# slp-rl/aero

Hardware: NVIDIA H100
Metric: audio-seconds/sec forward (higher is better)
Workload: dtype f16 tensor-core operands and activation storage (10-bit mantissa = tf32), fp32 accumulate / norm inputs / cell state

## Files before the change

aero_b200/csrc/tapgemm.cuh:

```cuda
#pragma once
#include <cuda.h>
#include "common.cuh"

namespace aero {
struct TapGemmArgs {
    const void* a1;
    const void* a2;
    const void* w;
    const float* bias;
    const float* addend_fn;
    const float* colscale;
    const void* residual;
    const float* samp_affine;
    void* out;
    double* stats;
    aero_tapgemm_params p;
    int ntaps;
    int tiles_t;
    int ldw;
    int vec_a;
    int vec_o;
    int vec_o8;
    uint32_t dv_mul[3], dv_shr[3];
    int direct_f16;
    int direct_f32;
    int last_tile;
};
constexpr int kBM = 128;
constexpr int kMaxStages = 8;
constexpr int kMaxBN = 128;
constexpr int kWideBN = 256;
constexpr int kSliceBN = 64;
constexpr int kProducerRegs = 40, kConsumerRegs = 232;
constexpr int kEpiWarps = 8;
constexpr int kThreads = 128 + 32 * kEpiWarps;
constexpr int kATileBytes = kBM * 128;

struct TcShared {
    uint64_t full[kMaxStages];
    uint64_t empty[kMaxStages];
    float stats[kEpiWarps][8][2];
    float part[kEpiWarps][4][2];
    alignas(16) float stage[kEpiWarps][32][20];
};

using KernelFn = void (*)(CUtensorMap, CUtensorMap, CUtensorMap, TapGemmArgs, int, int, int);
int tapgemm_simt_launch(const TapGemmArgs& g, cudaStream_t st);
int tapgemm_tc_launch(const TapGemmArgs& g, cudaStream_t st);
bool tapgemm_tc_eligible(const aero_tapgemm_params& p);
}
```

aero_b200/csrc/tapgemm_tc.cu:

```cuda
#include <cuda.h>
#include <mutex>
#include <unordered_map>
#include <string>
#include <cstring>
#include <cstdlib>

#include "tapgemm.cuh"
#include "tc_common.cuh"

namespace aero {

KernelFn tapgemm_tc_kernels_bn32(bool f16a, bool f16o, int amode, bool res, bool stats);
KernelFn tapgemm_tc_kernels_bn64(bool f16a, bool f16o, int amode, bool res, bool stats);
KernelFn tapgemm_tc_kernels_bn96(bool f16a, bool f16o, int amode, bool res, bool stats);
KernelFn tapgemm_tc_kernels_bn128(bool f16a, bool f16o, int amode, bool res, bool stats);
KernelFn tapgemm_tc_kernels_bn192(bool f16a, bool f16o, int amode, bool res, bool stats);
KernelFn tapgemm_tc_kernels_bn256(bool f16a, bool f16o, int amode, bool res, bool stats);

typedef CUresult (*EncodeTiledFn)(CUtensorMap*, CUtensorMapDataType, cuuint32_t, void*, const cuuint64_t*, const cuuint64_t*,
                                  const cuuint32_t*, const cuuint32_t*, CUtensorMapInterleave, CUtensorMapSwizzle,
                                  CUtensorMapL2promotion, CUtensorMapFloatOOBfill);

static EncodeTiledFn get_encode() {
    static EncodeTiledFn fn = nullptr;
// ... 18 lines not shown
    size_t operator()(const MapKey& k) const {
        const uint64_t* w = reinterpret_cast<const uint64_t*>(&k);
        size_t h = 1469598103934665603ull;
        for (size_t i = 0; i < sizeof(MapKey) / 8; ++i) h = (h ^ w[i]) * 1099511628211ull;
        return h;
    }
};

int encode_map(CUtensorMap* out, const void* base, uint32_t rank, const uint64_t* dims, const uint64_t* strides_bytes,
               const uint32_t* box, int swizzle_mode, int elem_bytes) {
    static std::mutex mu;
    static std::unordered_map<MapKey, CUtensorMap, MapKeyHash> cache;
    MapKey key;
    std::memset(&key, 0, sizeof(key));
    key.base = base;
    key.rank = rank;
    key.swz = (uint32_t)swizzle_mode | ((uint32_t)elem_bytes << 8);
    for (uint32_t i = 0; i < rank; ++i) { key.d[i] = dims[i]; key.box[i] = box[i]; }
    for (uint32_t i = 0; i + 1 < rank; ++i) key.s[i] = strides_bytes[i];
    {
        std::lock_guard<std::mutex> lk(mu);
        auto it = cache.find(key);
        if (it != cache.end()) { *out = it->second; return AERO_OK; }
    }
    EncodeTiledFn enc = get_encode();
    if (!enc) { set_error("cuTensorMapEncodeTiled not available from the driver"); return AERO_ERR_UNSUPPORTED; }
    cuuint64_t gd[4];
    cuuint64_t gs[3];
    cuuint32_t bx[4], es[4];
    for (uint32_t i = 0; i < rank; ++i) { gd[i] = dims[i]; bx[i] = box[i]; es[i] = 1; }
    for (uint32_t i = 0; i + 1 < rank; ++i) gs[i] = strides_bytes[i];
    CUresult r = enc(out, elem_bytes == 2 ? CU_TENSOR_MAP_DATA_TYPE_FLOAT16 : CU_TENSOR_MAP_DATA_TYPE_FLOAT32, rank, const_cast<void*>(base), gd, gs, bx, es,
                     CU_TENSOR_MAP_INTERLEAVE_NONE,
                     swizzle_mode == 2 ? CU_TENSOR_MAP_SWIZZLE_64B : CU_TENSOR_MAP_SWIZZLE_128B,
                     CU_TENSOR_MAP_L2_PROMOTION_L2_256B,
                     CU_TENSOR_MAP_FLOAT_OOB_FILL_NONE);
    if (r != CUDA_SUCCESS) {
        set_error("cuTensorMapEncodeTiled failed (%d): rank %u dims %llu %llu %llu %llu", (int)r, rank,
                  (unsigned long long)dims[0], (unsigned long long)dims[1], (unsigned long long)(rank > 2 ? dims[2] : 0),
                  (unsigned long long)(rank > 3 ? dims[3] : 0));
        return AERO_ERR_INVALID;
    }
    std::lock_guard<std::mutex> lk(mu);
    if (cache.size() > 4096) cache.clear();
    cache.emplace(key, *out);
    return AERO_OK;
}

static int tc_fixed_smem(int N, int BN) {
    return (int)sizeof(TcShared) + cdiv(N, BN) * BN * 4 + kBM * ((BN > kMaxBN ? kSliceBN : BN) + 4) * 4 + 1024;
}
static int tc_stages(int N, int BN) {
    if (N > (1 << 20)) return 0;
    const int st = (227 * 1024 - tc_fixed_smem(N, BN)) / (kATileBytes + BN * 128);
    return st > kMaxStages ? kMaxStages : st;
}

constexpr int kWideMinKTaps = 512;

static int pick_bn(const aero_tapgemm_params& p) {
    const int nt = cdiv(p.N, kMaxBN);
    const int narrow = (cdiv(p.N, nt) + 31) & ~31;
    if (p.precision != 2 || p.mode == AERO_TAPS_MIX || p.N < 192) return narrow;
    const int taps = (p.mode == AERO_TAPS_CONV) ? p.kf * p.kt : p.kf / p.stride_f;
    if ((int64_t)(p.C1 + p.C2) * taps < kWideMinKTaps) return narrow;
    const int bn = cdiv(p.N, cdiv(p.N, kWideBN)) <= 192 ? 192 : 256;
    if (tc_stages(p.N, bn) < 3) return narrow;
    if (p.stats_mode == 1) {
        const int Nout = p.glu ? p.N / 2 : p.N;
        if (p.groups < 1 || Nout % p.groups || (p.glu ? bn / 2 : bn) / (Nout / p.groups) + 2 > 8) return narrow;
    }
    return bn;
}

bool tapgemm_tc_eligible(const aero_tapgemm_params& p) {
    const bool f16 = (p.flags & AERO_TG_A_F16) != 0;
    const int q = f16 ? 8 : 4;
    if (p.mode == AERO_TAPS_MIX)
        return p.w_sb == 0 && p.C1 % q == 0 && p.C2 == 0 && p.a1_st % q == 0 && p.a1_sb % q == 0 && p.N >= 8 &&
               p.stats_mode == 0 && !p.glu && p.F_out == 1 && p.F_in == 1 && tc_stages(p.N, pick_bn(p)) >= 2;
    if (p.w_sb != 0) return false;
    if (p.act == AERO_ACT_TANH) return false;
    if (p.act == AERO_ACT_LEAKY && (p.stats_mode != 0 || p.r_sb != 0 || p.r_sf != 0 || p.r_st != 0))
        return false;
    if (tc_stages(p.N, pick_bn(p)) < 2) return false;
    if (p.N < 8) return false;
    const int K = p.C1 + p.C2;
    if (K < 8 || (p.C1 % q) || (p.C2 % q)) return false;
    auto ok_strides = [q](int64_t sb, int64_t sf, int64_t st) { return sb % q == 0 && sf % q == 0 && st % q == 0 && st > 0; };
    if (p.C1 && !ok_strides(p.a1_sb, p.a1_sf, p.a1_st)) return false;
    if (p.C2 && !ok_strides(p.a2_sb, p.a2_sf, p.a2_st)) return false;
    if (p.stats_mode == 1) {
        const int Nout = p.glu ? p.N / 2 : p.N;
        if (p.groups < 1 || Nout % p.groups) return false;
        const int gw = Nout / p.groups;
        const int bn = pick_bn(p);
        if (gw % 8 || (p.glu ? bn / 2 : bn) / gw + 2 > 8) return false;
    }
    return true;
}

static int make_a_map(CUtensorMap* m, const void* base, int C, const aero_tapgemm_params& p, int64_t sb, int64_t sf, int64_t st, int esz) {
    uint64_t dims[4] = {(uint64_t)C, (uint64_t)p.T_in, (uint64_t)p.F_in, (uint64_t)p.B};
    int64_t s1 = st, s2 = sf, s3 = sb;
    if (s2 <= 0) s2 = s1 * p.T_in;
    if (s3 <= 0) s3 = s2 * p.F_in;
    uint64_t strides[3] = {(uint64_t)s1 * esz, (uint64_t)s2 * esz, (uint64_t)s3 * esz};
    uint32_t box[4] = {(uint32_t)(128 / esz), (uint32_t)kBM, 1, 1};
    return encode_map(m, base, 4, dims, strides, box, 0, esz);
}

struct TcKnobs {
    int direct_f32 = -1, direct_f16 = -1, stages = -1;
    TcKnobs() {
        auto rd = [](const char* name, int& v) { if (const char* e = getenv(name)) v = atoi(e); };
        rd("AERO_TC_DIRECT_F32", direct_f32); rd("AERO_TC_DIRECT_F16", direct_f16); rd("AERO_TC_STAGES", stages);
    }
};
static const TcKnobs& knobs() { static const TcKnobs k; return k; }

int tapgemm_tc_launch(const TapGemmArgs& g0, cudaStream_t st) {
    const TcKnobs& kn = knobs();
    TapGemmArgs g = g0;
    const aero_tapgemm_params& p = g.p;
    const bool f16a = p.precision == 2, f16o = (p.flags & AERO_TG_OUT_F16) != 0;
    const int esz = f16a ? 2 : 4, kBKc = 128 / esz;
    const int K = p.C1 + p.C2;
    const int BN = pick_bn(p);
    const int nslab = (p.mode == AERO_TAPS_CONVT) ? p.kf : p.kf * p.kt;
    CUtensorMap mA1, mA2, mW;
    int rc;
    const bool mix = p.mode == AERO_TAPS_MIX;
    if (mix) {
        uint64_t dims[3] = {(uint64_t)p.T, (uint64_t)p.C1, (uint64_t)p.B};
        uint64_t strides[2] = {(uint64_t)p.a1_st * esz, (uint64_t)(p.a1_sb > 0 ? p.a1_sb : (int64_t)p.a1_st * p.C1) * esz};
        uint32_t box[3] = {(uint32_t)(f16a ? 64 : 32), (uint32_t)kBKc, 1};
        if ((rc = encode_map(&mA1, g.a1, 3, dims, strides, box, 0, esz)) != AERO_OK) return rc;
    } else if (p.C1) { if ((rc = make_a_map(&mA1, g.a1, p.C1, p, p.a1_sb, p.a1_sf, p.a1_st, esz)) != AERO_OK) return rc; }
    if (p.C2) { if ((rc = make_a_map(&mA2, g.a2, p.C2, p, p.a2_sb, p.a2_sf, p.a2_st, esz)) != AERO_OK) return rc; }
    if (!p.C1) mA1 = mA2;
    if (!p.C2) mA2 = mA1;
    {
        const uint64_t npad = (uint64_t)((p.N + 3) & ~3);
        const uint64_t kp = f16a ? (uint64_t)((K + 7) & ~7) : (uint64_t)K;
        uint64_t dims[3] = {(uint64_t)K, npad, (uint64_t)nslab};
        uint64_t strides[2] = {kp * esz, kp * npad * esz};
        uint32_t box[3] = {(uint32_t)kBKc, (uint32_t)BN, 1};
        if ((rc = encode_map(&mW, g.w, 3, dims, strides, box, 0, esz)) != AERO_OK) return rc;
    }
    g.tiles_t = cdiv(p.T, kBM);
    g.direct_f32 = 0;
    g.direct_f16 = 2;
    if (kn.direct_f32 >= 0) g.direct_f32 = kn.direct_f32;
    if (kn.direct_f16 >= 0) g.direct_f16 = kn.direct_f16;
    const int64_t tiles = (int64_t)p.B * p.F_out * g.tiles_t;
    if (tiles > 2147483647LL) { set_error("aero_tapgemm_fwd: too many tiles"); return AERO_ERR_INVALID; }
    {
        const uint32_t divs[3] = {(uint32_t)cdiv(p.N, BN), (uint32_t)g.tiles_t, (uint32_t)p.F_out};
        for (int i = 0; i < 3; ++i) {
            uint32_t s = 0;
            while ((1ull << s) < divs[i]) ++s;
            const uint64_t two = 1ull << (31 + s);
            g.dv_mul[i] = (uint32_t)((two + divs[i] - 1) / divs[i]);
            g.dv_shr[i] = 31 + s;
        }
    }
    const int stage_bytes = kATileBytes + BN * 128;
    const int fixed = tc_fixed_smem(p.N, BN);
    int kStages = tc_stages(p.N, BN);
    if (kStages < 2) {
        set_error("aero_tapgemm_fwd(wgmma): N = %d leaves no shared memory for the pipeline", p.N);
        return AERO_ERR_UNSUPPORTED;
    }
    if (kn.stages >= 2 && kn.stages < kStages) kStages = kn.stages;
    const size_t smem = (size_t)kStages * stage_bytes + fixed;
    const int amode = p.glu ? 3 : (p.act == AERO_ACT_LEAKY ? 4 : p.act);
    if (p.glu && p.act != AERO_ACT_NONE) { set_error("aero_tapgemm_fwd(wgmma): GLU with an activation is not supported"); return AERO_ERR_UNSUPPORTED; }
    const bool res = g.residual != nullptr, stats = p.stats_mode != 0;
    const KernelFn kern = BN == 32 ? tapgemm_tc_kernels_bn32(f16a, f16o, amode, res, stats)
                        : BN == 64 ? tapgemm_tc_kernels_bn64(f16a, f16o, amode, res, stats)
                        : BN == 96 ? tapgemm_tc_kernels_bn96(f16a, f16o, amode, res, stats)
                        : BN == 128 ? tapgemm_tc_kernels_bn128(f16a, f16o, amode, res, stats)
                        : BN == 192 ? tapgemm_tc_kernels_bn192(f16a, f16o, amode, res, stats)
                                    : tapgemm_tc_kernels_bn256(f16a, f16o, amode, res, stats);
    if (!kern) {
        set_error("aero_tapgemm_fwd(wgmma): epilogue (act %d, residual %d, stats %d) is not built for operands %s / outputs %s",
                  amode, (int)res, (int)stats, f16a ? "f16" : "tf32", f16o ? "f16" : "f32");
        return AERO_ERR_UNSUPPORTED;
    }
    cudaFuncSetAttribute(kern, cudaFuncAttributeMaxDynamicSharedMemorySize, 227 * 1024);
    static int num_sms = 0;
    if (num_sms == 0) {
        int dev = 0;
        cudaGetDevice(&dev);
        cudaDeviceGetAttribute(&num_sms, cudaDevAttrMultiProcessorCount, dev);
    }
    const int n_tiles = cdiv(p.N, BN);
    const int64_t tiles_total = tiles * n_tiles;
    if (tiles_total > 2147483647LL) { set_error("aero_tapgemm_fwd: too many tiles"); return AERO_ERR_INVALID; }
    const int64_t want = num_sms;
    g.last_tile = (int)tiles_total - 1;
    dim3 grid((unsigned)(tiles_total < want ? tiles_total : want));
    kern<<<grid, kThreads, smem, st>>>(mA1, mA2, mW, g, kStages, n_tiles, (int)tiles_total);
    return check_launch("aero_tapgemm_fwd(wgmma)");
}

}
```

aero_b200/csrc/tapgemm_tc_kernel.cuh:

```cuda
#pragma once
#include <cuda.h>
#include <type_traits>

#include "tapgemm.cuh"
#include "tc_common.cuh"


namespace aero {

template <bool F16A> struct OperandKind { static constexpr int kBK = F16A ? 64 : 32; };

struct TapIter {
    int fi, dt, slab;
};
__device__ __forceinline__ bool tap_geometry(const aero_tapgemm_params& p, int tap, int fo, TapIter& it) {
    if (p.mode == AERO_TAPS_CONV) {
        const int jf = tap / p.kt, jt = tap - jf * p.kt;
        it.fi = fo * p.stride_f + jf - p.pad_f;
        it.dt = jt * p.dil_t - p.pad_t;
        it.slab = tap;
    } else {
        const int fof = fo + p.f_out_offset;
        it.fi = fof / p.stride_f - tap;
        it.dt = 0;
        it.slab = fof % p.stride_f + tap * p.stride_f;
    }
    return it.fi >= 0 && it.fi < p.F_in;
}

struct TileCoord {
    int b, fo, t0, n0, n_iters;
};
__device__ __forceinline__ int fast_div(int n, uint32_t mul, uint32_t shr) {
    return (int)(((uint64_t)(uint32_t)n * mul) >> shr);
}
__device__ __forceinline__ int valid_taps(const aero_tapgemm_params& p, int fo, int ntaps) {
    if (p.mode == AERO_TAPS_CONV) {
        const int base = fo * p.stride_f - p.pad_f;
        const int lo = max(0, -base), hi = min(p.kf - 1, p.F_in - 1 - base);
        return max(0, hi - lo + 1) * p.kt;
    }
    const int a = (fo + p.f_out_offset) / p.stride_f;
    const int lo = max(0, a - p.F_in + 1), hi = min(ntaps - 1, a);
    return max(0, hi - lo + 1);
}
__device__ __forceinline__ TileCoord tile_coord(const TapGemmArgs& g, int tile, int n_tiles, int BN, int nch1, int nch2) {
    const aero_tapgemm_params& p = g.p;
    TileCoord c;
    if (p.flags & AERO_TG_REVERSE) tile = g.last_tile - tile;
    const int mt = fast_div(tile, g.dv_mul[0], g.dv_shr[0]), nt = tile - mt * n_tiles;
    const int row = fast_div(mt, g.dv_mul[1], g.dv_shr[1]), tt = mt - row * g.tiles_t;
    c.b = fast_div(row, g.dv_mul[2], g.dv_shr[2]);
    c.fo = row - c.b * p.F_out;
    c.t0 = tt * kBM;
    c.n0 = nt * BN;
    c.n_iters = (p.mode == AERO_TAPS_MIX) ? nch1 : valid_taps(p, c.fo, g.ntaps) * (nch1 + nch2);
    return c;
}

template <int AMODE>
__device__ __forceinline__ void epilogue_stage_a(const uint32_t (&r)[16], uint32_t stg_row, uint32_t sbias) {
    float4 bv[4];
#pragma unroll
    for (int j = 0; j < 4; ++j) bv[j] = lds128(sbias + 16 * j);
#pragma unroll
    for (int j = 0; j < 16; j += 4) {
        float v[4] = {__uint_as_float(r[j]) + bv[j / 4].x, __uint_as_float(r[j + 1]) + bv[j / 4].y,
                      __uint_as_float(r[j + 2]) + bv[j / 4].z, __uint_as_float(r[j + 3]) + bv[j / 4].w};
#pragma unroll
        for (int u = 0; u < 4; ++u) {
            if (AMODE == 1) v[u] = gelu_exact(v[u]);
            else if (AMODE == 2) v[u] = fmaxf(v[u], 0.f);
            else if (AMODE == 4) v[u] = leaky_f(v[u]);
        }
        if (AMODE == 3) {
            sts64(stg_row + (j / 2) * 4, v[0] * sigmoid_f(v[1]), v[2] * sigmoid_f(v[3]));
        } else {
            sts128(stg_row + j * 4, make_float4(v[0], v[1], v[2], v[3]));
        }
    }
}

template <int AMODE, bool RES, bool STATS, typename TO>
__device__ __forceinline__ void epilogue_fast_tile(TcShared* sh, const TapGemmArgs& g, const TileCoord& tc, uint32_t tacc, int c_lo, int c_hi,
                                                   int q, int ew, int lane, int Nout, int gw, int c_start, int c_step, uint32_t sbias) {
    const aero_tapgemm_params& p = g.p;
    constexpr int CNT = (AMODE == 3) ? 8 : 16;
    constexpr int LPR = CNT / 4;
    constexpr int RPI = 32 / LPR;
// ... 167 lines not shown
                    }
            } else {
#pragma unroll
                for (int j = 0; j < CNT; j += 4)
                    if (j < n_ok) *reinterpret_cast<float4*>(orow + no0 + j) = make_float4(o[j], o[j + 1], o[j + 2], o[j + 3]);
            }
        }
        if (STATS) {
#pragma unroll
            for (int j = 0; j < CNT; j += 4) {
                if (j < n_ok) {
                    const int gi = (no0 + j) / gw;
                    if (gi != cur_g) {
                        if (cur_g >= 0) {
                            const float a = warp_sum(ssum), c = warp_sum(ssq);
                            if (lane == 0) { sh->stats[ew][cur_g - g_lo][0] += a; sh->stats[ew][cur_g - g_lo][1] += c; }
                        }
                        cur_g = gi; ssum = 0.f; ssq = 0.f;
                    }
                    if (row_ok) {
                        ssum += (o[j] + o[j + 1]) + (o[j + 2] + o[j + 3]);
                        ssq += (o[j] * o[j] + o[j + 1] * o[j + 1]) + (o[j + 2] * o[j + 2] + o[j + 3] * o[j + 3]);
                    }
                }
            }
        }
    }
    if (STATS && cur_g >= 0) {
        const float a = warp_sum(ssum), c = warp_sum(ssq);
        if (lane == 0) { sh->stats[ew][cur_g - g_lo][0] += a; sh->stats[ew][cur_g - g_lo][1] += c; }
    }
}

template <int BN, bool F16A>
__device__ __forceinline__ void tile_mainloop(TcShared* sh, uint8_t* smem, int& stage, uint32_t& phase, const int kStages, const int stage_bytes,
                                              const int n_iters, const bool mix, const int wg, float (&d)[BN / 2]) {
    const int tid = threadIdx.x & 127, wl = tid >> 5, lane = tid & 31;
    int prev = -1;
    for (int i = 0; i < n_iters; ++i) {
        mbar_wait(&sh->full[stage], phase);
        const uint32_t sa = smem_u32(smem + stage * stage_bytes);
        const uint64_t db = make_desc_sw128(sa + kATileBytes);
        wgmma_fence();
        if (mix && F16A) {
            if constexpr (F16A) {
                const uint32_t sw = sa + (uint32_t)wg * 8192u;
                const uint64_t da = (uint64_t)((sw >> 4) & 0x3FFF) | ((uint64_t)(8192 >> 4) << 16) | ((uint64_t)(1024 >> 4) << 32) | ((uint64_t)1 << 62);
#pragma unroll
                for (int k = 0; k < 4; ++k) Wgmma<BN, true, 1>::ss(d, da + (uint64_t)(k * (2048 >> 4)), db + 2 * k, (i > 0 || k > 0) ? 1u : 0u);
            }
        } else if (mix) {
            if constexpr (!F16A) {
                const int m = wg * 64 + wl * 16 + (lane >> 2), c = lane & 3;
#pragma unroll
                for (int k = 0; k < 4; ++k) {
                    uint32_t a[4];
#pragma unroll
                    for (int u = 0; u < 4; ++u) {
                        const int mm = m + (u & 1) * 8, kk = 8 * k + c + (u >> 1) * 4;
                        const uint32_t addr = sa + (uint32_t)((mm >> 5) * 4096 + kk * 128 + ((((mm & 31) >> 2) ^ (kk & 7)) << 4) + ((mm & 3) << 2));
                        asm volatile("ld.shared.b32 %0, [%1];" : "=r"(a[u]) : "r"(addr));
                    }
                    Wgmma<BN, false, 0>::rs(d, a, db + 2 * k, (i > 0 || k > 0) ? 1u : 0u);
                }
            }
        } else {
            const uint64_t da = make_desc_sw128(sa + (uint32_t)wg * (64 * 128));
#pragma unroll
            for (int k = 0; k < 4; ++k)
                Wgmma<BN, F16A, 0>::ss(d, da + 2 * k, db + 2 * k, (i > 0 || k > 0) ? 1u : 0u);
        }
        wgmma_commit();
        wgmma_wait<1>();
        if (prev >= 0 && tid == 0) mbar_arrive(&sh->empty[prev]);
        prev = stage;
        if (++stage == kStages) { stage = 0; phase ^= 1; }
    }
    wgmma_wait<0>();
    if (prev >= 0 && tid == 0) mbar_arrive(&sh->empty[prev]);
}

template <int BN, int SW>
__device__ __forceinline__ void stage_acc(const float (&d)[BN / 2], const int s0, float* acc, const int wg) {
    constexpr int ldacc = SW + 4;
    const int tid = threadIdx.x & 127, wl = tid >> 5, lane = tid & 31;
    float* row = acc + (wg * 64 + wl * 16 + (lane >> 2)) * ldacc + 2 * (lane & 3);
#pragma unroll
    for (int j = 0; j < SW / 8; ++j) {
        const int jd = s0 / 8 + j;
        *reinterpret_cast<float2*>(row + 8 * j) = make_float2(d[4 * jd], d[4 * jd + 1]);
        *reinterpret_cast<float2*>(row + 8 * ldacc + 8 * j) = make_float2(d[4 * jd + 2], d[4 * jd + 3]);
    }
}

template <int BN, int AMODE, bool RES, bool STATS, bool F16A, bool F16O>
__global__ void __launch_bounds__(kThreads, 1)
tapgemm_tc_kernel(const __grid_constant__ CUtensorMap mapA1, const __grid_constant__ CUtensorMap mapA2,
                  const __grid_constant__ CUtensorMap mapW, const TapGemmArgs g, const int kStages, const int n_tiles,
                  const int tiles_total) {
    extern __shared__ uint8_t smem_raw[];
    uint8_t* smem = reinterpret_cast<uint8_t*>((reinterpret_cast<uintptr_t>(smem_raw) + 1023) & ~(uintptr_t)1023);
    constexpr int stage_bytes = kATileBytes + BN * 128;
    TcShared* sh = reinterpret_cast<TcShared*>(smem + kStages * stage_bytes);
    float* const sbias_f = reinterpret_cast<float*>(sh + 1);
    const uint32_t sbias = smem_u32(sbias_f);
    constexpr bool kWide = BN > kMaxBN;
    constexpr int kSW = kWide ? kSliceBN : BN;
    float* const acc = sbias_f + n_tiles * BN;
    constexpr int ldacc = kSW + 4;

    using TO = typename std::conditional<F16O, __half, float>::type;
    constexpr int kBKc = OperandKind<F16A>::kBK;
    const aero_tapgemm_params& p = g.p;
    const int warp = threadIdx.x >> 5, lane = threadIdx.x & 31;
    const int nch1 = (p.C1 + kBKc - 1) / kBKc, nch2 = (p.C2 + kBKc - 1) / kBKc;
    const bool mix = !kWide && p.mode == AERO_TAPS_MIX;

    for (int i = threadIdx.x; i < n_tiles * BN; i += kThreads) sbias_f[i] = (g.bias && i < g.p.N) ? g.bias[i] : 0.f;
    if (threadIdx.x == 0) {
        for (int s = 0; s < kStages; ++s) { mbar_init(&sh->full[s], 1); mbar_init(&sh->empty[s], 2); }
        asm volatile("fence.mbarrier_init.release.cluster;" ::: "memory");
        for (int w = 0; w < kEpiWarps; ++w)
            for (int i = 0; i < 8; ++i) { sh->stats[w][i][0] = 0.f; sh->stats[w][i][1] = 0.f; }
    }
    __syncthreads();

    if (warp < 4) {
        if constexpr (kWide) asm volatile("setmaxnreg.dec.sync.aligned.u32 %0;" ::"n"(kProducerRegs));
        if (warp == 0 && lane == 0) {
            asm volatile("prefetch.tensormap [%0];" ::"l"(&mapA1) : "memory");
            asm volatile("prefetch.tensormap [%0];" ::"l"(&mapW) : "memory");
            int stage = 0;
            uint32_t phase = 0;
            const uint32_t tx = (uint32_t)stage_bytes;
            int ptl = 0;
            for (int tile = blockIdx.x; tile < tiles_total; tile += gridDim.x, ++ptl) {
                const TileCoord c = tile_coord(g, tile, n_tiles, BN, nch1, nch2);
                if (mix) {
                    for (int kc = 0; kc < nch1; ++kc) {
                        mbar_wait(&sh->empty[stage], phase ^ 1);
                        uint8_t* sa = smem + stage * stage_bytes;
                        mbar_expect_tx(&sh->full[stage], tx);
                        constexpr int kBoxM = F16A ? 64 : 32;
#pragma unroll
                        for (int j = 0; j < 128 / kBoxM; ++j)
                            tma_load_3d(sa + j * (kATileBytes / (128 / kBoxM)), &mapA1, &sh->full[stage], c.t0 + kBoxM * j, kc * kBKc, c.b);
                        tma_load_3d(sa + kATileBytes, &mapW, &sh->full[stage], kc * kBKc, c.n0, 0);
                        if (++stage == kStages) { stage = 0; phase ^= 1; }
                    }
                    continue;
                }
                for (int tap = 0; tap < g.ntaps; ++tap) {
                    TapIter it;
                    if (!tap_geometry(p, tap, c.fo, it)) continue;
                    for (int src = 0; src < 2; ++src) {
                        const int nch = src ? nch2 : nch1;
                        const CUtensorMap* mA = src ? &mapA2 : &mapA1;
                        const int kw0 = src ? p.C1 : 0;
                        for (int kc = 0; kc < nch; ++kc) {
                            mbar_wait(&sh->empty[stage], phase ^ 1);
                            uint8_t* sa = smem + stage * stage_bytes;
                            mbar_expect_tx(&sh->full[stage], tx);
                            tma_load_4d(sa, mA, &sh->full[stage], kc * kBKc, c.t0 + it.dt, it.fi, c.b);
                            tma_load_3d(sa + kATileBytes, &mapW, &sh->full[stage], kw0 + kc * kBKc, c.n0, it.slab);
                            if (++stage == kStages) { stage = 0; phase ^= 1; }
                        }
                    }
                }
            }
        }
    } else {
        if constexpr (kWide) asm volatile("setmaxnreg.inc.sync.aligned.u32 %0;" ::"n"(kConsumerRegs));
        const int wg = (warp >> 2) - 1;
        const int ew = warp - 4;
        const int q = 2 * wg + (warp & 1);
        const int grp = (warp >> 1) & 1;
        const int m = q * 32 + lane;
        const int Nout = p.glu ? p.N / 2 : p.N;
        const int gw = (p.stats_mode == 1) ? Nout / p.groups : Nout;
        const bool rnd = (p.flags & 1) && !F16O;
        const int c_start = grp * 16, c_step = 32;
        const bool fast = !mix && g.vec_o && !g.colscale && (p.stats_mode == 0 || gw % 4 == 0);
        int stage = 0, local = 0;
        uint32_t phase = 0;
        for (int tile = blockIdx.x; tile < tiles_total; tile += gridDim.x, ++local) {
            const TileCoord tc = tile_coord(g, tile, n_tiles, BN, nch1, nch2);
            const int b = tc.b, fo = tc.fo, t0 = tc.t0, n0 = tc.n0, n_iters = tc.n_iters;
            const int g_lo = (p.glu ? n0 >> 1 : n0) / gw;
            float d[BN / 2];
            tile_mainloop<BN, F16A>(sh, smem, stage, phase, kStages, stage_bytes, n_iters, mix, wg, d);
#pragma unroll
            for (int s0 = 0; s0 < BN; s0 += kSW) {
                if (s0 > 0) warpgroup_sync(1 + wg);
                stage_acc<BN, kSW>(d, s0, acc, wg);
                warpgroup_sync(1 + wg);
                const uint32_t tacc = smem_u32(acc + m * ldacc);
                const int t = t0 + m;
                const bool row_ok = t < p.T;
                float sa = 1.f, sb = 0.f;
                if (g.samp_affine) { sa = g.samp_affine[2 * b]; sb = g.samp_affine[2 * b + 1]; }
                TO* op = static_cast<TO*>(g.out) + (int64_t)b * p.o_sb + (int64_t)fo * p.o_sf + (int64_t)t * p.o_st;
                const TO* rp = g.residual ? static_cast<const TO*>(g.residual) + (int64_t)b * p.r_sb + (int64_t)fo * p.r_sf + (int64_t)t * p.r_st : nullptr;
                const float* csp = g.colscale ? g.colscale + (int64_t)b * p.cs_sb + (int64_t)t * p.cs_st : nullptr;
                const float* adp = g.addend_fn ? g.addend_fn + (int64_t)fo * Nout : nullptr;
                int cur_g = -1;
                float ssum = 0.f, ssq = 0.f;

                if (mix) {
                    const float gate = (row_ok && g.colscale) ? g.colscale[(int64_t)b * p.cs_sb + t] : 1.f;
                    TO* ob = static_cast<TO*>(g.out) + (int64_t)b * p.o_sb + t;
                    for (int c0 = c_start; c0 < BN; c0 += c_step) {
                        uint32_t r[16];
                        acc_ld16(tacc + 4u * (uint32_t)c0, r);
                        if (row_ok) {
#pragma unroll
                            for (int j = 0; j < 16; ++j) {
                                const int n = n0 + c0 + j;
                                if (n < p.N) {
                                    float x = __uint_as_float(r[j]) * gate;
                                    if (rnd) x = round_tf32_rna(x);
                                    stf(ob + (int64_t)n * p.o_st, x);
                                }
                            }
// ... 154 lines not shown
```

aero_b200/csrc/wgmma.cuh:

```cuda
#pragma once
#include <cstdint>

namespace aero {

__device__ __forceinline__ void wgmma_fence() { asm volatile("wgmma.fence.sync.aligned;" ::: "memory"); }
__device__ __forceinline__ void wgmma_commit() { asm volatile("wgmma.commit_group.sync.aligned;" ::: "memory"); }
template <int PENDING>
__device__ __forceinline__ void wgmma_wait() { asm volatile("wgmma.wait_group.sync.aligned %0;" ::"n"(PENDING) : "memory"); }

template <int ROWB>
__device__ __forceinline__ uint64_t make_desc_kmajor(uint32_t saddr) {
    return (uint64_t)((saddr >> 4) & 0x3FFF) | ((uint64_t)1 << 16) | ((uint64_t)((ROWB * 8) >> 4) << 32) |
           ((uint64_t)(ROWB == 128 ? 1 : 2) << 62);
}
__device__ __forceinline__ uint64_t make_desc_sw128(uint32_t saddr) { return make_desc_kmajor<128>(saddr); }

template <int N, bool F16, int TA> struct Wgmma;

template <int TA> struct Wgmma<8, true, TA> {
    static __device__ __forceinline__ void rs(float (&d)[4], const uint32_t (&a)[4], uint64_t db, uint32_t acc) {
        asm volatile("{\n\t.reg .pred p;\n\tsetp.ne.b32 p, %9, 0;\n\t"
                     "wgmma.mma_async.sync.aligned.m64n8k16.f32.f16.f16 {%0, %1, %2, %3}, {%4, %5, %6, %7}, %8, p, 1, 1, 0;\n\t}"
            : "+f"(d[0]), "+f"(d[1]), "+f"(d[2]), "+f"(d[3])
            : "r"(a[0]), "r"(a[1]), "r"(a[2]), "r"(a[3]), "l"(db), "r"(acc));
    }
};
template <int TA> struct Wgmma<16, true, TA> {
    static __device__ __forceinline__ void ss(float (&d)[8], uint64_t da, uint64_t db, uint32_t acc) {
        asm volatile("{\n\t.reg .pred p;\n\tsetp.ne.b32 p, %10, 0;\n\t"
                     "wgmma.mma_async.sync.aligned.m64n16k16.f32.f16.f16 {%0, %1, %2, %3, %4, %5, %6, %7}, %8, %9, p, 1, 1, %11, 0;\n\t}"
            : "+f"(d[0]), "+f"(d[1]), "+f"(d[2]), "+f"(d[3]), "+f"(d[4]), "+f"(d[5]), "+f"(d[6]), "+f"(d[7])
            : "l"(da), "l"(db), "r"(acc), "n"(TA));
    }
    static __device__ __forceinline__ void rs(float (&d)[8], const uint32_t (&a)[4], uint64_t db, uint32_t acc) {
        asm volatile("{\n\t.reg .pred p;\n\tsetp.ne.b32 p, %13, 0;\n\t"
                     "wgmma.mma_async.sync.aligned.m64n16k16.f32.f16.f16 {%0, %1, %2, %3, %4, %5, %6, %7}, {%8, %9, %10, %11}, %12, p, 1, 1, 0;\n\t}"
            : "+f"(d[0]), "+f"(d[1]), "+f"(d[2]), "+f"(d[3]), "+f"(d[4]), "+f"(d[5]), "+f"(d[6]), "+f"(d[7])
            : "r"(a[0]), "r"(a[1]), "r"(a[2]), "r"(a[3]), "l"(db), "r"(acc));
    }
};
template <> struct Wgmma<16, false, 0> {
    static __device__ __forceinline__ void ss(float (&d)[8], uint64_t da, uint64_t db, uint32_t acc) {
        asm volatile("{\n\t.reg .pred p;\n\tsetp.ne.b32 p, %10, 0;\n\t"
                     "wgmma.mma_async.sync.aligned.m64n16k8.f32.tf32.tf32 {%0, %1, %2, %3, %4, %5, %6, %7}, %8, %9, p, 1, 1;\n\t}"
            : "+f"(d[0]), "+f"(d[1]), "+f"(d[2]), "+f"(d[3]), "+f"(d[4]), "+f"(d[5]), "+f"(d[6]), "+f"(d[7])
            : "l"(da), "l"(db), "r"(acc));
// ... 300 lines not shown
```

Measured before the change: 3740.

## Use narrower swizzled TMA boxes and trimmed WGMMA k-steps for partial channel chunks

Adds 32B and 64B swizzle tensor maps alongside the 128B ones for both activations and weights. The last K-chunk of each source now loads only the bytes it needs and issues only the WGMMA k-steps covering real channels. Stage size is derived from the widest box actually used, so layers whose channel counts fit in narrow rows get more pipeline stages. The aim is to stop paying for the zero padding of partial chunks in TMA traffic and tensor-core work. The cost is extra kernel parameters, branching on row width in the mainloop, and a per-chunk expected-transaction size that must stay consistent with the loads.

Result: no change. 3727, median of 6 (-0.3%).

```diff
diff --git a/aero_b200/csrc/tapgemm.cuh b/aero_b200/csrc/tapgemm.cuh
--- a/aero_b200/csrc/tapgemm.cuh
+++ b/aero_b200/csrc/tapgemm.cuh
@@ -25,6 +25,7 @@
     int direct_f16;
     int direct_f32;
     int last_tile;
+    int nch1, nch2, last1, last2, stage_bytes;
 };
 constexpr int kBM = 128;
 constexpr int kMaxStages = 8;
@@ -44,7 +45,25 @@
     alignas(16) float stage[kEpiWarps][32][20];
 };
 
-using KernelFn = void (*)(CUtensorMap, CUtensorMap, CUtensorMap, TapGemmArgs, int, int, int);
+__host__ __device__ inline int tc_last_row_bytes(int C, int esz) {
+    const int r = (C * esz) & 127;
+    return r ? (r + 31) & ~31 : 128;
+}
+__host__ __device__ inline int tc_box_bytes(int rb) { return rb <= 32 ? 32 : rb <= 64 ? 64 : 128; }
+__host__ __device__ inline int tc_box_widths(int C, int esz) {
+    if (C <= 0) return 0;
+    const int box = tc_box_bytes(tc_last_row_bytes(C, esz));
+    return (C * esz >= 128 || box == 128 ? 1 : 0) | (box == 64 ? 2 : 0) | (box == 32 ? 4 : 0);
+}
+__host__ __device__ inline int tc_slot_row_bytes(int C1, int C2, int esz) {
+    const int w = tc_box_widths(C1, esz) | tc_box_widths(C2, esz);
+    return (w & 1) ? 128 : (w & 2) ? 64 : 32;
+}
+struct TcMaps {
+    CUtensorMap a[2][3];
+    CUtensorMap w[3];
+};
+using KernelFn = void (*)(TcMaps, TapGemmArgs, int, int, int);
 int tapgemm_simt_launch(const TapGemmArgs& g, cudaStream_t st);
 int tapgemm_tc_launch(const TapGemmArgs& g, cudaStream_t st);
 bool tapgemm_tc_eligible(const aero_tapgemm_params& p);
diff --git a/aero_b200/csrc/tapgemm_tc.cu b/aero_b200/csrc/tapgemm_tc.cu
--- a/aero_b200/csrc/tapgemm_tc.cu
+++ b/aero_b200/csrc/tapgemm_tc.cu
@@ -74,7 +74,7 @@
     for (uint32_t i = 0; i + 1 < rank; ++i) gs[i] = strides_bytes[i];
     CUresult r = enc(out, elem_bytes == 2 ? CU_TENSOR_MAP_DATA_TYPE_FLOAT16 : CU_TENSOR_MAP_DATA_TYPE_FLOAT32, rank, const_cast<void*>(base), gd, gs, bx, es,
                      CU_TENSOR_MAP_INTERLEAVE_NONE,
-                     swizzle_mode == 2 ? CU_TENSOR_MAP_SWIZZLE_64B : CU_TENSOR_MAP_SWIZZLE_128B,
+                     swizzle_mode == 3 ? CU_TENSOR_MAP_SWIZZLE_32B : swizzle_mode == 2 ? CU_TENSOR_MAP_SWIZZLE_64B : CU_TENSOR_MAP_SWIZZLE_128B,
                      CU_TENSOR_MAP_L2_PROMOTION_L2_256B,
                      CU_TENSOR_MAP_FLOAT_OOB_FILL_NONE);
     if (r != CUDA_SUCCESS) {
@@ -92,9 +92,12 @@
 static int tc_fixed_smem(int N, int BN) {
     return (int)sizeof(TcShared) + cdiv(N, BN) * BN * 4 + kBM * ((BN > kMaxBN ? kSliceBN : BN) + 4) * 4 + 1024;
 }
-static int tc_stages(int N, int BN) {
+static int tc_row_bytes(const aero_tapgemm_params& p) {
+    return p.mode == AERO_TAPS_MIX ? 128 : tc_slot_row_bytes(p.C1, p.C2, p.precision == 2 ? 2 : 4);
+}
+static int tc_stages(int N, int BN, int row_bytes) {
     if (N > (1 << 20)) return 0;
-    const int st = (227 * 1024 - tc_fixed_smem(N, BN)) / (kATileBytes + BN * 128);
+    const int st = (227 * 1024 - tc_fixed_smem(N, BN)) / ((kBM + BN) * row_bytes);
     return st > kMaxStages ? kMaxStages : st;
 }
 
@@ -107,7 +110,7 @@
     const int taps = (p.mode == AERO_TAPS_CONV) ? p.kf * p.kt : p.kf / p.stride_f;
     if ((int64_t)(p.C1 + p.C2) * taps < kWideMinKTaps) return narrow;
     const int bn = cdiv(p.N, cdiv(p.N, kWideBN)) <= 192 ? 192 : 256;
-    if (tc_stages(p.N, bn) < 3) return narrow;
+    if (tc_stages(p.N, bn, tc_row_bytes(p)) < 3) return narrow;
     if (p.stats_mode == 1) {
         const int Nout = p.glu ? p.N / 2 : p.N;
         if (p.groups < 1 || Nout % p.groups || (p.glu ? bn / 2 : bn) / (Nout / p.groups) + 2 > 8) return narrow;
@@ -120,12 +123,12 @@
     const int q = f16 ? 8 : 4;
     if (p.mode == AERO_TAPS_MIX)
         return p.w_sb == 0 && p.C1 % q == 0 && p.C2 == 0 && p.a1_st % q == 0 && p.a1_sb % q == 0 && p.N >= 8 &&
-               p.stats_mode == 0 && !p.glu && p.F_out == 1 && p.F_in == 1 && tc_stages(p.N, pick_bn(p)) >= 2;
+               p.stats_mode == 0 && !p.glu && p.F_out == 1 && p.F_in == 1 && tc_stages(p.N, pick_bn(p), 128) >= 2;
     if (p.w_sb != 0) return false;
     if (p.act == AERO_ACT_TANH) return false;
     if (p.act == AERO_ACT_LEAKY && (p.stats_mode != 0 || p.r_sb != 0 || p.r_sf != 0 || p.r_st != 0))
         return false;
-    if (tc_stages(p.N, pick_bn(p)) < 2) return false;
+    if (tc_stages(p.N, pick_bn(p), tc_row_bytes(p)) < 2) return false;
     if (p.N < 8) return false;
     const int K = p.C1 + p.C2;
     if (K < 8 || (p.C1 % q) || (p.C2 % q)) return false;
@@ -142,14 +145,17 @@
     return true;
 }
 
-static int make_a_map(CUtensorMap* m, const void* base, int C, const aero_tapgemm_params& p, int64_t sb, int64_t sf, int64_t st, int esz) {
+static const int kBoxBytes[3] = {128, 64, 32}, kBoxSwizzle[3] = {0, 2, 3};
+
+static int make_a_map(CUtensorMap* m, const void* base, int C, const aero_tapgemm_params& p, int64_t sb, int64_t sf, int64_t st, int esz,
+                      int wi) {
     uint64_t dims[4] = {(uint64_t)C, (uint64_t)p.T_in, (uint64_t)p.F_in, (uint64_t)p.B};
     int64_t s1 = st, s2 = sf, s3 = sb;
     if (s2 <= 0) s2 = s1 * p.T_in;
     if (s3 <= 0) s3 = s2 * p.F_in;
     uint64_t strides[3] = {(uint64_t)s1 * esz, (uint64_t)s2 * esz, (uint64_t)s3 * esz};
-    uint32_t box[4] = {(uint32_t)(128 / esz), (uint32_t)kBM, 1, 1};
-    return encode_map(m, base, 4, dims, strides, box, 0, esz);
+    uint32_t box[4] = {(uint32_t)(kBoxBytes[wi] / esz), (uint32_t)kBM, 1, 1};
+    return encode_map(m, base, 4, dims, strides, box, kBoxSwizzle[wi], esz);
 }
 
 struct TcKnobs {
@@ -170,25 +176,39 @@
     const int K = p.C1 + p.C2;
     const int BN = pick_bn(p);
     const int nslab = (p.mode == AERO_TAPS_CONVT) ? p.kf : p.kf * p.kt;
-    CUtensorMap mA1, mA2, mW;
+    TcMaps maps;
+    std::memset(&maps, 0, sizeof(maps));
     int rc;
     const bool mix = p.mode == AERO_TAPS_MIX;
+    int w_widths = 1;
     if (mix) {
         uint64_t dims[3] = {(uint64_t)p.T, (uint64_t)p.C1, (uint64_t)p.B};
         uint64_t strides[2] = {(uint64_t)p.a1_st * esz, (uint64_t)(p.a1_sb > 0 ? p.a1_sb : (int64_t)p.a1_st * p.C1) * esz};
         uint32_t box[3] = {(uint32_t)(f16a ? 64 : 32), (uint32_t)kBKc, 1};
-        if ((rc = encode_map(&mA1, g.a1, 3, dims, strides, box, 0, esz)) != AERO_OK) return rc;
-    } else if (p.C1) { if ((rc = make_a_map(&mA1, g.a1, p.C1, p, p.a1_sb, p.a1_sf, p.a1_st, esz)) != AERO_OK) return rc; }
-    if (p.C2) { if ((rc = make_a_map(&mA2, g.a2, p.C2, p, p.a2_sb, p.a2_sf, p.a2_st, esz)) != AERO_OK) return rc; }
-    if (!p.C1) mA1 = mA2;
-    if (!p.C2) mA2 = mA1;
+        if ((rc = encode_map(&maps.a[0][0], g.a1, 3, dims, strides, box, 0, esz)) != AERO_OK) return rc;
+    } else {
+        const void* base[2] = {g.a1, g.a2};
+        const int C[2] = {p.C1, p.C2};
+        const int64_t s[2][3] = {{p.a1_sb, p.a1_sf, p.a1_st}, {p.a2_sb, p.a2_sf, p.a2_st}};
+        w_widths = 0;
+        for (int src = 0; src < 2; ++src) {
+            const int widths = tc_box_widths(C[src], esz);
+            w_widths |= widths;
+            for (int wi = 0; wi < 3; ++wi)
+                if ((widths >> wi & 1) &&
+                    (rc = make_a_map(&maps.a[src][wi], base[src], C[src], p, s[src][0], s[src][1], s[src][2], esz, wi)) != AERO_OK)
+                    return rc;
+        }
+    }
     {
         const uint64_t npad = (uint64_t)((p.N + 3) & ~3);
         const uint64_t kp = f16a ? (uint64_t)((K + 7) & ~7) : (uint64_t)K;
         uint64_t dims[3] = {(uint64_t)K, npad, (uint64_t)nslab};
         uint64_t strides[2] = {kp * esz, kp * npad * esz};
-        uint32_t box[3] = {(uint32_t)kBKc, (uint32_t)BN, 1};
-        if ((rc = encode_map(&mW, g.w, 3, dims, strides, box, 0, esz)) != AERO_OK) return rc;
+        for (int wi = 0; wi < 3; ++wi) {
+            uint32_t box[3] = {(uint32_t)(kBoxBytes[wi] / esz), (uint32_t)BN, 1};
+            if ((w_widths >> wi & 1) && (rc = encode_map(&maps.w[wi], g.w, 3, dims, strides, box, kBoxSwizzle[wi], esz)) != AERO_OK) return rc;
+        }
     }
     g.tiles_t = cdiv(p.T, kBM);
     g.direct_f32 = 0;
@@ -207,9 +227,14 @@
             g.dv_shr[i] = 31 + s;
         }
     }
-    const int stage_bytes = kATileBytes + BN * 128;
+    g.nch1 = cdiv(p.C1, kBKc);
+    g.nch2 = mix ? 0 : cdiv(p.C2, kBKc);
+    g.last1 = mix ? 128 : tc_last_row_bytes(p.C1, esz);
+    g.last2 = mix ? 128 : tc_last_row_bytes(p.C2, esz);
+    g.stage_bytes = (kBM + BN) * tc_row_bytes(p);
+    const int stage_bytes = g.stage_bytes;
     const int fixed = tc_fixed_smem(p.N, BN);
-    int kStages = tc_stages(p.N, BN);
+    int kStages = tc_stages(p.N, BN, tc_row_bytes(p));
     if (kStages < 2) {
         set_error("aero_tapgemm_fwd(wgmma): N = %d leaves no shared memory for the pipeline", p.N);
         return AERO_ERR_UNSUPPORTED;
@@ -243,7 +268,7 @@
     const int64_t want = num_sms;
     g.last_tile = (int)tiles_total - 1;
     dim3 grid((unsigned)(tiles_total < want ? tiles_total : want));
-    kern<<<grid, kThreads, smem, st>>>(mA1, mA2, mW, g, kStages, n_tiles, (int)tiles_total);
+    kern<<<grid, kThreads, smem, st>>>(maps, g, kStages, n_tiles, (int)tiles_total);
     return check_launch("aero_tapgemm_fwd(wgmma)");
 }
 
diff --git a/aero_b200/csrc/tapgemm_tc_kernel.cuh b/aero_b200/csrc/tapgemm_tc_kernel.cuh
--- a/aero_b200/csrc/tapgemm_tc_kernel.cuh
+++ b/aero_b200/csrc/tapgemm_tc_kernel.cuh
@@ -29,7 +29,7 @@
 }
 
 struct TileCoord {
-    int b, fo, t0, n0, n_iters;
+    int b, fo, t0, n0, taps, n_iters;
 };
 __device__ __forceinline__ int fast_div(int n, uint32_t mul, uint32_t shr) {
     return (int)(((uint64_t)(uint32_t)n * mul) >> shr);
@@ -44,7 +44,7 @@
     const int lo = max(0, a - p.F_in + 1), hi = min(ntaps - 1, a);
     return max(0, hi - lo + 1);
 }
-__device__ __forceinline__ TileCoord tile_coord(const TapGemmArgs& g, int tile, int n_tiles, int BN, int nch1, int nch2) {
+__device__ __forceinline__ TileCoord tile_coord(const TapGemmArgs& g, int tile, int n_tiles, int BN) {
     const aero_tapgemm_params& p = g.p;
     TileCoord c;
     if (p.flags & AERO_TG_REVERSE) tile = g.last_tile - tile;
@@ -54,7 +54,8 @@
     c.fo = row - c.b * p.F_out;
     c.t0 = tt * kBM;
     c.n0 = nt * BN;
-    c.n_iters = (p.mode == AERO_TAPS_MIX) ? nch1 : valid_taps(p, c.fo, g.ntaps) * (nch1 + nch2);
+    c.taps = (p.mode == AERO_TAPS_MIX) ? 1 : valid_taps(p, c.fo, g.ntaps);
+    c.n_iters = c.taps * (g.nch1 + g.nch2);
     return c;
 }
 
@@ -288,52 +289,94 @@
     }
 }
 
+template <int BN, bool F16A, bool MIX>
+__device__ __forceinline__ void mainloop_stage(TcShared* sh, uint8_t* smem, int& stage, uint32_t& phase, int& prev, const int kStages,
+                                               const int stage_bytes, const int rb, const bool first, const int wg, float (&d)[BN / 2]) {
+    const int tid = threadIdx.x & 127, wl = tid >> 5, lane = tid & 31;
+    mbar_wait(&sh->full[stage], phase);
+    const uint32_t sa = smem_u32(smem + stage * stage_bytes);
+    const uint32_t w0 = (uint32_t)tc_box_bytes(rb);
+    const uint64_t da = make_desc_kmajor(sa + (uint32_t)wg * 64u * w0, w0), db = make_desc_kmajor(sa + (uint32_t)kBM * w0, w0);
+    const uint32_t sw = sa + (uint32_t)wg * 8192u;
+    const uint64_t dm = (uint64_t)((sw >> 4) & 0x3FFF) | ((uint64_t)(8192 >> 4) << 16) | ((uint64_t)(1024 >> 4) << 32) | ((uint64_t)1 << 62);
+    const uint32_t acc0 = first ? 0u : 1u;
+    uint32_t af[MIX && !F16A ? 4 : 1][4];
+    if constexpr (MIX && !F16A) {
+        const int m = wg * 64 + wl * 16 + (lane >> 2), c = lane & 3;
+#pragma unroll
+        for (int k = 0; k < 4; ++k)
+#pragma unroll
+            for (int u = 0; u < 4; ++u) {
+                const int mm = m + (u & 1) * 8, kk = 8 * k + c + (u >> 1) * 4;
+                const uint32_t addr = sa + (uint32_t)((mm >> 5) * 4096 + kk * 128 + ((((mm & 31) >> 2) ^ (kk & 7)) << 4) + ((mm & 3) << 2));
+                asm volatile("ld.shared.b32 %0, [%1];" : "=r"(af[k][u]) : "r"(addr));
+            }
+    }
+    wgmma_fence();
+    if constexpr (MIX && F16A) {
+#pragma unroll
+        for (int k = 0; k < 4; ++k) Wgmma<BN, true, 1>::ss(d, dm + (uint64_t)(k * (2048 >> 4)), db + 2 * k, k > 0 ? 1u : acc0);
+        wgmma_commit();
+    } else if constexpr (MIX) {
+#pragma unroll
+        for (int k = 0; k < 4; ++k) Wgmma<BN, false, 0>::rs(d, af[k], db + 2 * k, k > 0 ? 1u : acc0);
+        wgmma_commit();
+    } else if (rb == 128) {
+#pragma unroll
+        for (int k = 0; k < 4; ++k) Wgmma<BN, F16A, 0>::ss(d, da + 2 * k, db + 2 * k, k > 0 ? 1u : acc0);
+        wgmma_commit();
+    } else if (rb == 96) {
+#pragma unroll
+        for (int k = 0; k < 3; ++k) Wgmma<BN, F16A, 0>::ss(d, da + 2 * k, db + 2 * k, k > 0 ? 1u : acc0);
+        wgmma_commit();
+    } else if (rb == 64) {
+        Wgmma<BN, F16A, 0>::ss(d, da, db, acc0);
+        Wgmma<BN, F16A, 0>::ss(d, da + 2, db + 2, 1u);
+        wgmma_commit();
+    } else {
+        Wgmma<BN, F16A, 0>::ss(d, da, db, acc0);
+        wgmma_commit();
+    }
+    if constexpr (MIX && !F16A) wgmma_wait<0>();
+    else wgmma_wait<1>();
+    if (prev >= 0 && tid == 0) mbar_arrive(&sh->empty[prev]);
+    prev = stage;
+    if (++stage == kStages) { stage = 0; phase ^= 1; }
+}
+
 template <int BN, bool F16A>
-__device__ __forceinline__ void tile_mainloop(TcShared* sh, uint8_t* smem, int& stage, uint32_t& phase, const int kStages, const int stage_bytes,
-                                              const int n_iters, const bool mix, const int wg, float (&d)[BN / 2]) {
-    const int tid = threadIdx.x & 127, wl = tid >> 5, lane = tid & 31;
+__device__ __forceinline__ void tile_mainloop(TcShared* sh, uint8_t* smem, int& stage, uint32_t& phase, const int kStages, const TapGemmArgs& g,
+                                              const int taps, const bool mix, const int wg, float (&d)[BN / 2]) {
+    const int stage_bytes = g.stage_bytes;
     int prev = -1;
-    for (int i = 0; i < n_iters; ++i) {
-        mbar_wait(&sh->full[stage], phase);
-        const uint32_t sa = smem_u32(smem + stage * stage_bytes);
-        const uint64_t db = make_desc_sw128(sa + kATileBytes);
-        wgmma_fence();
-        if (mix && F16A) {
-            if constexpr (F16A) {
-                const uint32_t sw = sa + (uint32_t)wg * 8192u;
-                const uint64_t da = (uint64_t)((sw >> 4) & 0x3FFF) | ((uint64_t)(8192 >> 4) << 16) | ((uint64_t)(1024 >> 4) << 32) | ((uint64_t)1 << 62);
-#pragma unroll
-                for (int k = 0; k < 4; ++k) Wgmma<BN, true, 1>::ss(d, da + (uint64_t)(k * (2048 >> 4)), db + 2 * k, (i > 0 || k > 0) ? 1u : 0u);
-            }
-        } else if (mix) {
-            if constexpr (!F16A) {
-                const int m = wg * 64 + wl * 16 + (lane >> 2), c = lane & 3;
-#pragma unroll
-                for (int k = 0; k < 4; ++k) {
-                    uint32_t a[4];
-#pragma unroll
-                    for (int u = 0; u < 4; ++u) {
-                        const int mm = m + (u & 1) * 8, kk = 8 * k + c + (u >> 1) * 4;
-                        const uint32_t addr = sa + (uint32_t)((mm >> 5) * 4096 + kk * 128 + ((((mm & 31) >> 2) ^ (kk & 7)) << 4) + ((mm & 3) << 2));
-                        asm volatile("ld.shared.b32 %0, [%1];" : "=r"(a[u]) : "r"(addr));
-                    }
-                    Wgmma<BN, false, 0>::rs(d, a, db + 2 * k, (i > 0 || k > 0) ? 1u : 0u);
-                }
-            }
-        } else {
-            const uint64_t da = make_desc_sw128(sa + (uint32_t)wg * (64 * 128));
-#pragma unroll
-            for (int k = 0; k < 4; ++k)
-                Wgmma<BN, F16A, 0>::ss(d, da + 2 * k, db + 2 * k, (i > 0 || k > 0) ? 1u : 0u);
-        }
-        wgmma_commit();
-        wgmma_wait<1>();
-        if (prev >= 0 && tid == 0) mbar_arrive(&sh->empty[prev]);
-        prev = stage;
-        if (++stage == kStages) { stage = 0; phase ^= 1; }
+    bool first = true;
+    if (mix) {
+        for (int kc = 0; kc < g.nch1; ++kc) {
+            mainloop_stage<BN, F16A, true>(sh, smem, stage, phase, prev, kStages, stage_bytes, 128, first, wg, d);
+            first = false;
+        }
+    } else if (g.last1 == 128 && g.last2 == 128) {
+        for (int i = 0; i < taps * (g.nch1 + g.nch2); ++i) {
+            mainloop_stage<BN, F16A, false>(sh, smem, stage, phase, prev, kStages, stage_bytes, 128, first, wg, d);
+            first = false;
+        }
+    } else {
+        for (int t = 0; t < taps; ++t) {
+#pragma unroll
+            for (int s = 0; s < 2; ++s) {
+                const int nch = s ? g.nch2 : g.nch1;
+                if (nch == 0) continue;
+                for (int kc = 0; kc < nch - 1; ++kc) {
+                    mainloop_stage<BN, F16A, false>(sh, smem, stage, phase, prev, kStages, stage_bytes, 128, first, wg, d);
+                    first = false;
+                }
+                mainloop_stage<BN, F16A, false>(sh, smem, stage, phase, prev, kStages, stage_bytes, s ? g.last2 : g.last1, first, wg, d);
+                first = false;
+            }
+        }
     }
     wgmma_wait<0>();
-    if (prev >= 0 && tid == 0) mbar_arrive(&sh->empty[prev]);
+    if (prev >= 0 && (threadIdx.x & 127) == 0) mbar_arrive(&sh->empty[prev]);
 }
 
 template <int BN, int SW>
@@ -351,26 +394,24 @@
 
 template <int BN, int AMODE, bool RES, bool STATS, bool F16A, bool F16O>
 __global__ void __launch_bounds__(kThreads, 1)
-tapgemm_tc_kernel(const __grid_constant__ CUtensorMap mapA1, const __grid_constant__ CUtensorMap mapA2,
-                  const __grid_constant__ CUtensorMap mapW, const TapGemmArgs g, const int kStages, const int n_tiles,
-                  const int tiles_total) {
+tapgemm_tc_kernel(const __grid_constant__ TcMaps maps, const TapGemmArgs g, const int kStages, const int n_tiles, const int tiles_total) {
     extern __shared__ uint8_t smem_raw[];
     uint8_t* smem = reinterpret_cast<uint8_t*>((reinterpret_cast<uintptr_t>(smem_raw) + 1023) & ~(uintptr_t)1023);
-    constexpr int stage_bytes = kATileBytes + BN * 128;
+    constexpr bool kWide = BN > kMaxBN;
+    constexpr int kEsz = F16A ? 2 : 4;
+    const aero_tapgemm_params& p = g.p;
+    const bool mix = !kWide && p.mode == AERO_TAPS_MIX;
+    const int stage_bytes = g.stage_bytes;
     TcShared* sh = reinterpret_cast<TcShared*>(smem + kStages * stage_bytes);
     float* const sbias_f = reinterpret_cast<float*>(sh + 1);
     const uint32_t sbias = smem_u32(sbias_f);
-    constexpr bool kWide = BN > kMaxBN;
     constexpr int kSW = kWide ? kSliceBN : BN;
     float* const acc = sbias_f + n_tiles * BN;
     constexpr int ldacc = kSW + 4;
 
     using TO = typename std::conditional<F16O, __half, float>::type;
     constexpr int kBKc = OperandKind<F16A>::kBK;
-    const aero_tapgemm_params& p = g.p;
     const int warp = threadIdx.x >> 5, lane = threadIdx.x & 31;
-    const int nch1 = (p.C1 + kBKc - 1) / kBKc, nch2 = (p.C2 + kBKc - 1) / kBKc;
-    const bool mix = !kWide && p.mode == AERO_TAPS_MIX;
 
     for (int i = threadIdx.x; i < n_tiles * BN; i += kThreads) sbias_f[i] = (g.bias && i < g.p.N) ? g.bias[i] : 0.f;
     if (threadIdx.x == 0) {
@@ -384,24 +425,27 @@
     if (warp < 4) {
         if constexpr (kWide) asm volatile("setmaxnreg.dec.sync.aligned.u32 %0;" ::"n"(kProducerRegs));
         if (warp == 0 && lane == 0) {
-            asm volatile("prefetch.tensormap [%0];" ::"l"(&mapA1) : "memory");
-            asm volatile("prefetch.tensormap [%0];" ::"l"(&mapW) : "memory");
+            const int widths[2] = {mix ? 1 : tc_box_widths(p.C1, kEsz), mix ? 0 : tc_box_widths(p.C2, kEsz)};
+            for (int wi = 0; wi < 3; ++wi) {
+                for (int s = 0; s < 2; ++s)
+                    if (widths[s] >> wi & 1) asm volatile("prefetch.tensormap [%0];" ::"l"(&maps.a[s][wi]) : "memory");
+                if ((widths[0] | widths[1]) >> wi & 1) asm volatile("prefetch.tensormap [%0];" ::"l"(&maps.w[wi]) : "memory");
+            }
             int stage = 0;
             uint32_t phase = 0;
-            const uint32_t tx = (uint32_t)stage_bytes;
             int ptl = 0;
             for (int tile = blockIdx.x; tile < tiles_total; tile += gridDim.x, ++ptl) {
-                const TileCoord c = tile_coord(g, tile, n_tiles, BN, nch1, nch2);
+                const TileCoord c = tile_coord(g, tile, n_tiles, BN);
                 if (mix) {
-                    for (int kc = 0; kc < nch1; ++kc) {
+                    for (int kc = 0; kc < g.nch1; ++kc) {
                         mbar_wait(&sh->empty[stage], phase ^ 1);
                         uint8_t* sa = smem + stage * stage_bytes;
-                        mbar_expect_tx(&sh->full[stage], tx);
+                        mbar_expect_tx(&sh->full[stage], (uint32_t)stage_bytes);
                         constexpr int kBoxM = F16A ? 64 : 32;
 #pragma unroll
                         for (int j = 0; j < 128 / kBoxM; ++j)
-                            tma_load_3d(sa + j * (kATileBytes / (128 / kBoxM)), &mapA1, &sh->full[stage], c.t0 + kBoxM * j, kc * kBKc, c.b);
-                        tma_load_3d(sa + kATileBytes, &mapW, &sh->full[stage], kc * kBKc, c.n0, 0);
+                            tma_load_3d(sa + j * (kATileBytes / (128 / kBoxM)), &maps.a[0][0], &sh->full[stage], c.t0 + kBoxM * j, kc * kBKc, c.b);
+                        tma_load_3d(sa + kATileBytes, &maps.w[0], &sh->full[stage], kc * kBKc, c.n0, 0);
                         if (++stage == kStages) { stage = 0; phase ^= 1; }
                     }
                     continue;
@@ -410,15 +454,17 @@
                     TapIter it;
                     if (!tap_geometry(p, tap, c.fo, it)) continue;
                     for (int src = 0; src < 2; ++src) {
-                        const int nch = src ? nch2 : nch1;
-                        const CUtensorMap* mA = src ? &mapA2 : &mapA1;
-                        const int kw0 = src ? p.C1 : 0;
+                        const int nch = src ? g.nch2 : g.nch1;
+                        const CUtensorMap* mA = maps.a[src];
+                        const int kw0 = src ? p.C1 : 0, last = src ? g.last2 : g.last1;
                         for (int kc = 0; kc < nch; ++kc) {
+                            const int rb = kc == nch - 1 ? last : 128;
+                            const int w = tc_box_bytes(rb), wi = w == 128 ? 0 : w == 64 ? 1 : 2;
                             mbar_wait(&sh->empty[stage], phase ^ 1);
                             uint8_t* sa = smem + stage * stage_bytes;
-                            mbar_expect_tx(&sh->full[stage], tx);
-                            tma_load_4d(sa, mA, &sh->full[stage], kc * kBKc, c.t0 + it.dt, it.fi, c.b);
-                            tma_load_3d(sa + kATileBytes, &mapW, &sh->full[stage], kw0 + kc * kBKc, c.n0, it.slab);
+                            mbar_expect_tx(&sh->full[stage], (uint32_t)((kBM + BN) * w));
+                            tma_load_4d(sa, &mA[wi], &sh->full[stage], kc * kBKc, c.t0 + it.dt, it.fi, c.b);
+                            tma_load_3d(sa + kBM * w, &maps.w[wi], &sh->full[stage], kw0 + kc * kBKc, c.n0, it.slab);
                             if (++stage == kStages) { stage = 0; phase ^= 1; }
                         }
                     }
@@ -440,11 +486,11 @@
         int stage = 0, local = 0;
         uint32_t phase = 0;
         for (int tile = blockIdx.x; tile < tiles_total; tile += gridDim.x, ++local) {
-            const TileCoord tc = tile_coord(g, tile, n_tiles, BN, nch1, nch2);
+            const TileCoord tc = tile_coord(g, tile, n_tiles, BN);
             const int b = tc.b, fo = tc.fo, t0 = tc.t0, n0 = tc.n0, n_iters = tc.n_iters;
             const int g_lo = (p.glu ? n0 >> 1 : n0) / gw;
             float d[BN / 2];
-            tile_mainloop<BN, F16A>(sh, smem, stage, phase, kStages, stage_bytes, n_iters, mix, wg, d);
+            tile_mainloop<BN, F16A>(sh, smem, stage, phase, kStages, g, tc.taps, mix, wg, d);
 #pragma unroll
             for (int s0 = 0; s0 < BN; s0 += kSW) {
                 if (s0 > 0) warpgroup_sync(1 + wg);
diff --git a/aero_b200/csrc/wgmma.cuh b/aero_b200/csrc/wgmma.cuh
--- a/aero_b200/csrc/wgmma.cuh
+++ b/aero_b200/csrc/wgmma.cuh
@@ -8,10 +8,14 @@
 template <int PENDING>
 __device__ __forceinline__ void wgmma_wait() { asm volatile("wgmma.wait_group.sync.aligned %0;" ::"n"(PENDING) : "memory"); }
 
+__device__ __forceinline__ uint64_t make_desc_kmajor(uint32_t saddr, uint32_t rowb) {
+    const uint64_t layout = rowb == 128 ? 1 : rowb == 64 ? 2 : 3;
+    return (uint64_t)((saddr >> 4) & 0x3FFF) | ((uint64_t)1 << 16) | ((uint64_t)((rowb * 8) >> 4) << 32) | (layout << 62);
+}
 template <int ROWB>
 __device__ __forceinline__ uint64_t make_desc_kmajor(uint32_t saddr) {
-    return (uint64_t)((saddr >> 4) & 0x3FFF) | ((uint64_t)1 << 16) | ((uint64_t)((ROWB * 8) >> 4) << 32) |
-           ((uint64_t)(ROWB == 128 ? 1 : 2) << 62);
+    static_assert(ROWB == 128 || ROWB == 64 || ROWB == 32, "swizzled K-major rows are 32, 64 or 128 bytes");
+    return make_desc_kmajor(saddr, (uint32_t)ROWB);
 }
 __device__ __forceinline__ uint64_t make_desc_sw128(uint32_t saddr) { return make_desc_kmajor<128>(saddr); }
 
```
